# saegsali/visual-odometry-project

Measured on AMD Instinct MI355X. Metric: VO frames/sec at 1376x1241, 2k keypoints; pose err vs reference, higher is better.
Workload: dtype f64

## Files before the change

### visual-odometry-project_amd/csrc/pipeline.h

```cpp
#pragma once

#include <linux/futex.h>
#include <sys/prctl.h>
#include <sys/syscall.h>
#include <time.h>
#include <unistd.h>

#include <atomic>
#include <chrono>
#include <cmath>
#include <cstdlib>
#include <string>
#include <mutex>
#include <thread>
#include <vector>

#include "vo_state.h"
#include "state_device.h"

struct vo_pipeline_boot;

struct vo_pipeline {
  vo_ctx* ctx = nullptr;
  vo_ctx* det = nullptr;
// ... 27 lines not shown
  struct lens_t {
    bool on = false, have_raw = false;
    double dist[5] = {0, 0, 0, 0, 0}, K_raw[9] = {0, 0, 0, 0, 0, 0, 0, 0, 0};
  };
  std::vector<lens_t> lens;
  uint8_t* d_raw[2] = {nullptr, nullptr};
  uint8_t* h_bgr = nullptr;
  hipEvent_t evBgr = nullptr;
  int prepared_idx = -1, prepared_slot = -1;
  int slot = 0, det_flip = 0, prev_frame = -1;
  vo_feat F[2];
  void* feat_mem = nullptr;
  int cur = 0;
  vo_seq_ctl* d_ctl = nullptr;
  float *d_next = nullptr, *d_err = nullptr;
  uint8_t* d_status = nullptr;
  double *d_R = nullptr, *d_t = nullptr;
  uint8_t* d_valid = nullptr;
  int32_t *d_counts = nullptr, *d_samples = nullptr, *d_pend = nullptr;
  uint64_t *d_masks = nullptr, *d_best_mask = nullptr;
  double* d_table = nullptr;
  std::vector<double> table;
  int table_len = 0;
  uint32_t* d_raws = nullptr;
  uint32_t ring_len = 0;
  uint32_t* h_stage = nullptr;
  size_t stage_cap = 0;
  std::vector<uint64_t> gen_upto, pos_known, pos_dev;
  std::vector<vo_pcg64> raw_gen, rng;
  hipEvent_t evRaw = nullptr;
  bool raw_pending = false, seeded = false, have_state = false, primed = false;
  vo_step_result *h_res = nullptr, *m_res = nullptr;
  volatile unsigned* h_seq = nullptr;
  unsigned* m_seq = nullptr;
  unsigned seq = 0;
  struct flight_t { int prev_idx = 0, next_idx = 0, a = 0, b = 0, fcur = 0, rslot = 0; unsigned seq = 0; long k = 0; unsigned front_job = 0; };
  flight_t flight[2];
  int n_flight = 0;
  long steps_submitted = 0;
  std::vector<unsigned> slot_seq;
  std::vector<char> seq_state;
  int last_fbuf = 0;
  long last_k = 0;
  int ckpt_par = 0;
  hipEvent_t evA = nullptr, evB = nullptr;
  double* d_newkp = nullptr;
// ... 134 lines not shown
```

### visual-odometry-project_amd/csrc/pipeline.hip

```cpp
#include "pipeline.h"

#pragma clang fp contract(off)

namespace {

hipError_t mset(hipStream_t st, void* dst, int v, size_t bytes) {
  hipError_t e = hipMemsetAsync(dst, v, bytes, st);
  return e != hipSuccess ? e : hipStreamSynchronize(st);
}

uint32_t next_pow2(uint64_t v) {
  uint32_t r = 1;
  while (r < v) r <<= 1;
  return r;
}

vo_feat carve(char*& q, int cap, int S, bool ids) {
  vo_feat f;
  auto take = [&](size_t bytes) {
    void* r = q;
    q += (bytes * S + 255) & ~size_t(255);
    return r;
  };
  f.kp = (float*)take((size_t)cap * 8);
// ... 160 lines not shown
  VO_REQUIRE(ctx, cfg->track_ids == 0 || cfg->track_ids == 1, "pipeline: track_ids must be 0 (off) or 1 (on), got %d", cfg->track_ids);
  VO_REQUIRE(ctx, cfg->detector == 0 || cfg->tracker_mode == 0,
             "pipeline: the Shi-Tomasi detector (detector = 1) belongs to the KLT tracker mode (tracker_mode = 0)");
  if (cfg->detector == 1) {
    const int rc = vo_good_features_batch_check(ctx, cfg->sequences > 0 ? cfg->sequences : 1, cfg->H, cfg->W,
                                                cfg->st_quality == 0.0 ? 0.01 : cfg->st_quality,
                                                cfg->st_min_distance == 0.0 ? 8.0 : cfg->st_min_distance,
                                                cfg->st_block == 0 ? 7 : cfg->st_block);
    if (rc != VO_OK) return rc;
  }
  const int cap = cfg->feature_cap > 0 ? cfg->feature_cap : 2 * cfg->n_keypoints;
  VO_REQUIRE(ctx, cap >= cfg->n_keypoints && cap <= 32768, "pipeline: feature_cap must be in n_keypoints..32768");
  VO_HIP_TRY(ctx, hipSetDevice(ctx->device));
  vo_pipeline* p = new (std::nothrow) vo_pipeline();
  if (!p) return VO_ENOMEM;
  p->ctx = ctx;
  p->cfg = *cfg;
  p->cap = cap;
  p->words = vo_cdiv(cap, 64);
  p->S = cfg->sequences > 0 ? cfg->sequences : 1;
  p->cfg.sequences = p->S;
  const int S = p->S;
  if (p->cfg.bearing_threshold == 0.0) p->cfg.bearing_threshold = 0.0075;
  if (p->cfg.redetect_fraction == 0.0) p->cfg.redetect_fraction = 0.8;
  if (p->cfg.detect_margin == 0.0) p->cfg.detect_margin = 0.01;
  if (p->cfg.detect_losses <= 0.0) p->cfg.detect_losses = 2.5;
  if (p->cfg.st_block == 0) p->cfg.st_block = 7;
  if (p->cfg.st_quality == 0.0) p->cfg.st_quality = 0.01;
  if (p->cfg.st_min_distance == 0.0) p->cfg.st_min_distance = 8.0;
  p->detect_losses = p->cfg.detect_losses;
  p->detect_limit = p->cfg.detect_margin < 0.0 ? -1.0 : p->cfg.redetect_fraction + p->cfg.detect_margin;
  if (p->cfg.debug_never_detect) p->detect_limit = 0.0;
  {
    bool given = false;
    for (double v : cfg->Kinv) given |= v != 0.0;
    p->cams.assign((size_t)p->S, make_cam(cfg->K, given ? cfg->Kinv : nullptr));
  }
  p->idle.assign((size_t)p->S, 0);
  memset(&p->seed_rng, 0, sizeof(p->seed_rng));
  int rc = VO_OK;
  void* side = getenv("VO_ONE_STREAM") ? (void*)ctx->stream : nullptr;
  {
    const char* sc = getenv("VO_SIDE_CUS");
    p->side_cfg = vo_stream_cfg_parse(sc, getenv("VO_STREAM_PRIORITY"));
    if (!sc && p->S <= 2 && p->detect_limit >= 0.0 && !side && cfg->tracker_mode == 0) {
      hipDeviceProp_t prop;
// ... 366 lines not shown
```

### visual-odometry-project_amd/csrc/pipeline_state.hip

```cpp
#include <algorithm>

#include "pipeline.h"

#pragma clang fp contract(off)

namespace {

struct pose17 {
  double v[17];
};

__global__ __launch_bounds__(256) void export_state_kernel(pose17 head, const double* __restrict__ land, int n, int cap,
                                                           double* __restrict__ rec) {
  const int i = blockIdx.x * blockDim.x + threadIdx.x;
  if (i < 17) rec[i] = head.v[i];
  const int m = min(n, cap) * 3;
  if (i < m) rec[17 + i] = land[i];
}

__global__ __launch_bounds__(256) void export_tracks_kernel(vo_feat F, const vo_seq_ctl* __restrict__ ctl, int slot, int n,
                                                            int cap, int seq, unsigned long long* __restrict__ rec) {
  const int i = blockIdx.x * 256 + threadIdx.x;
  auto pack = [](int lo, int hi) { return (unsigned long long)(unsigned)lo | ((unsigned long long)(unsigned)hi << 32); };
  if (i == 0) {
// ... 452 lines not shown
    VO_HIP_TRY(ctx, hipMemcpyAsync(p->d_newkp, new_kp, (size_t)n2 * 16, hipMemcpyHostToDevice, st));
    VO_HIP_TRY(ctx, hipMemcpyAsync(p->d_pairs, pairs, (size_t)M * 8, hipMemcpyHostToDevice, st));
    vo_pairs_batch bt;
    bt.par = (int)(p->steps_submitted & 1);
    VO_TRY(vo_state_regroup_pairs(ctx, p->d_ctl, p->F[p->cur], p->F[1 - p->cur], p->d_pairs, M, p->d_newkp, n2, p->cap, nullptr,
                                  nullptr, nullptr, 1, &bt));
    VO_HIP_TRY(ctx, hipStreamSynchronize(st));
    p->cur = 1 - p->cur;
    vo_seq_ctl h;
    VO_HIP_TRY(ctx, mcpy(st, &h, p->d_ctl, sizeof(h), hipMemcpyDeviceToHost));
    memcpy(h.T_in_wc, T_wc, 96);
    memcpy(h.T_in_cw, T_cw, 96);
    h.n_cand = h.n_dropped = h.n_land = h.done = 0;
    h.next_id[bt.par] = h.next_id[bt.par ^ 1];
    h.id_step[bt.par] = h.id_step[bt.par ^ 1];
    VO_HIP_TRY(ctx, mcpy(st, p->d_ctl, &h, sizeof(h), hipMemcpyHostToDevice));
    std::vector<uint64_t> bits((size_t)p->words, ~0ull);
    if (p3p_inliers)
      for (int i = 0; i < h.n_tri; ++i)
        if (!p3p_inliers[i]) bits[i >> 6] &= ~(1ull << (i & 63));
    VO_HIP_TRY(ctx, mcpy(st, p->d_best_mask, bits.data(), bits.size() * 8, hipMemcpyHostToDevice));
  }
  if (phases & 1)
    VO_TRY(vo_state_candidates(ctx, p->d_ctl, p->F[p->cur], p->d_best_mask, p->d_cams, p->cfg.bearing_threshold, -1, p->cap));
  if (phases & 2)
    VO_TRY(vo_state_landmarks(ctx, p->d_ctl, p->F[p->cur], p->d_cams, -1, p->cap, nullptr, nullptr, 0u));
  VO_HIP_TRY(ctx, hipStreamSynchronize(st));
  return VO_OK;
}

int vo_pipeline_export_state_post_seq(vo_pipeline* p, int seq, const vo_step_result* r, int cap, double* d_record) {
  if (!p || !r || !d_record) return VO_EINVAL;
  vo_ctx* ctx = p->ctx;
  VO_REQUIRE(ctx, cap >= 0 && seq >= 0 && seq < p->S, "pipeline_export_state: bad capacity or sequence index");
  pose17 h;
  for (int row = 0; row < 3; ++row) {
    for (int c = 0; c < 3; ++c) h.v[4 * row + c] = r->R_refined[3 * row + c];
    h.v[4 * row + 3] = r->t_refined[row];
  }
  h.v[12] = h.v[13] = h.v[14] = 0.0;
  h.v[15] = 1.0;
  const int n = r->best_index >= 0 ? (r->n_triangulated < cap ? r->n_triangulated : cap) : 0;
  h.v[16] = (double)n;
  const int threads = n * 3 > 17 ? n * 3 : 17;
  {
    vo_prof_scope ps(ctx, VO_K_EXPORT);
    hipLaunchKernelGGL(export_state_kernel, dim3(vo_cdiv(threads, 256)), dim3(256), 0, ctx->stream, h,
// ... 129 lines not shown
```

### visual-odometry-project_amd/csrc/pipeline_step.hip

```cpp
#include "pipeline.h"

#pragma clang fp contract(off)

namespace {

__global__ __launch_bounds__(64) void detect_decide_kernel(const vo_seq_ctl* __restrict__ ctl, int S, double limit, int n_det,
                                                           int force, int* __restrict__ go, double losses) {
  const int q = blockIdx.x * 64 + threadIdx.x;
  if (q >= S) return;
  if (ctl[q].fault & VO_FAULT_IDLE) {
    go[q] = 0;
    return;
  }
  const int n2 = ctl[q].n2;
  const int lost = max(ctl[q].n_in - (ctl[q].redetected ? (n_det < 0 ? ctl[q].num_features : n_det) : 0) - n2, 0);
  go[q] = (force || limit < 0.0 || (limit > 0.0 && (double)n2 - losses * (double)lost < (double)ctl[q].num_features * limit)) ? 1 : 0;
}

__global__ void ctl_resume_kernel(vo_seq_ctl* __restrict__ ctl) {
  ctl->fault = 0;
  ctl->n_p3p = ctl->n_tri;
}

__global__ __launch_bounds__(256) void sift_kp_f64_kernel(const float* __restrict__ rows, const int* __restrict__ n, int cap,
// ... 152 lines not shown
  p->gen_upto[q] = target;
  return VO_OK;
}

static vo_pose_job make_pose_job(vo_pipeline* p, const vo_feat& B, int do_replay, int q0) {
  const vo_pipeline_config& c = p->cfg;
  const size_t q = (size_t)q0;
  vo_pose_job j;
  j.ctl = p->d_ctl + q;
  j.rp.valid = p->d_valid + q * c.hyp;
  j.rp.counts = p->d_counts + q * c.hyp;
  j.rp.R = p->d_R + q * c.hyp * 9;
  j.rp.t = p->d_t + q * c.hyp * 3;
  j.rp.masks = (const unsigned long long*)p->d_masks + q * c.hyp * p->words;
  j.rp.words = p->words;
  j.rp.hyp = c.hyp;
  j.rp.table = p->d_table;
  j.rp.table_len = p->table_len;
  j.rp.max_it = c.ransac_max_iterations;
  j.rp.best_mask = (unsigned long long*)p->d_best_mask + q * p->words;
  j.do_replay = do_replay;
  j.B = vo_feat_seq(B, q);
  j.cam = p->d_cams + q;
  j.bearing_thr = c.bearing_threshold;
  j.max_iter = c.refine_iters;
  j.tail = 0;
  j.res = nullptr;
  j.seq_word = nullptr;
  j.seq = 0u;
  static const int stamps = getenv("VO_POSE_STAMPS") ? 1 : 0;
  j.stamps = stamps;
  j.debug_fault_every = 0;
  return j;
}

static int enqueue_tracker(vo_pipeline* p, const vo_pipeline::flight_t& f, bool with_pyramid, int q0, int Sn) {
  vo_ctx* ctx = p->ctx;
  const vo_pipeline_config& c = p->cfg;
  const vo_feat A = vo_feat_seq(p->F[f.fcur], (size_t)q0);
  hipStream_t ts = p->trk->stream;
  if (with_pyramid) VO_TRY(enqueue_pyramid(p, f.next_idx, f.b));
  if (f.k > 0 && hipEventQuery(p->evRegroup[(f.k - 1) & 1]) != hipSuccess)
    VO_HIP_TRY(ctx, hipStreamWaitEvent(ts, p->evRegroup[(f.k - 1) & 1], 0));
  if (hipEventQuery(p->evDet[f.a]) != hipSuccess) VO_HIP_TRY(ctx, hipStreamWaitEvent(ts, p->evDet[f.a], 0));
  vo_seq_ctl* ctl = p->d_ctl + q0;
  vo_klt_source src;
  src.n = &ctl->n2;
// ... 64 lines not shown
  const size_t q = (size_t)q0;
  const vo_feat B = vo_feat_seq(p->F[1 - f.fcur], q);
  vo_seq_ctl* ctl = p->d_ctl + q0;
  vo_hyp_batch hb;
  hb.S = Sn;
  hb.X = (size_t)p->cap * 3;
  hb.x = (size_t)p->cap * 2;
  hb.raws = p->ring_len;
  hb.ctl = sizeof(vo_seq_ctl);
  hb.cam = reinterpret_cast<const double*>(p->d_cams + q);
  hb.cam_stride = sizeof(vo_cam) / sizeof(double);
  VO_TRY(vo_p3p_hypotheses_ring_dev(ctx, B.land, B.kp64, &ctl->n_p3p, p->cap, c.K, p->d_raws + q * p->ring_len, &ctl->raw_pos,
                                    p->ring_len - 1, c.hyp, c.p3p_thr_sq, p->d_R + q * c.hyp * 9, p->d_t + q * c.hyp * 3,
                                    p->d_valid + q * c.hyp, p->d_counts + q * c.hyp, p->d_masks + q * c.hyp * p->words,
                                    (uint32_t*)&ctl->solve_flag, (uint64_t*)&ctl->ts[2], &hb));
  vo_pose_job job = make_pose_job(p, p->F[1 - f.fcur], 1, q0);
  job.walk = 0;
  job.res = p->m_res + (size_t)f.rslot * p->S + q;
  job.seq_word = p->m_seq + (size_t)f.rslot * p->S + q;
  job.seq = seq;
  job.debug_fault_every = debug_pose_fault;
  VO_TRY(vo_frame_pose(ctx, job, Sn));
  const uint64_t* bm = p->d_best_mask + (size_t)q0 * p->words;
  return vo_state_walk_landmarks(ctx, ctl, B, bm, p->words, p->d_cams + q0, c.bearing_threshold, c.refine_iters > 0 ? 1 : 0,
                                 p->cap, p->d_pend + q * p->cap, job.res, job.seq_word, seq, Sn);
}

extern "C" int vo_sift_dev(vo_ctx* ctx, const uint8_t* d_img, int H, int W, int cap, float* d_kp, float* d_desc,
                           uint8_t* d_desc_u8, int32_t* d_n);

static int enqueue_sift(vo_pipeline* p, const vo_pipeline::flight_t& f, char* err_buf = nullptr) {
  vo_ctx* sc = (f.k & 1) ? p->det : p->trk;
  const vo_pipeline_config& c = p->cfg;
  int rc = VO_OK;
  if (sc != p->trk && hipStreamWaitEvent(sc->stream, p->evImg[f.next_idx], 0) != hipSuccess) rc = VO_EHIP;
  if (rc == VO_OK && p->n_pinned[f.next_idx] > 0 && hipStreamWaitEvent(sc->stream, p->evUp[f.next_idx], 0) != hipSuccess) rc = VO_EHIP;
  if (rc == VO_OK && p->sift_all)
    rc = vo_sift_all_found_dev(sc, p->img(0, f.next_idx), p->img_stride(), 1, c.H, c.W, p->frame_rows,
                               p->d_skp + (size_t)f.b * p->frame_rows * 6, (size_t)p->frame_rows, nullptr, p->frame_desc(f.b, 0),
                               (size_t)p->frame_rows, p->frame_n(f.b, 0), p->d_sover + 2 * f.b, p->d_sover + 2 * f.b + 1);
  else if (rc == VO_OK)
    rc = vo_sift_dev(sc, p->img(0, f.next_idx), c.H, c.W, p->frame_rows, p->d_skp + (size_t)f.b * p->frame_rows * 6, nullptr,
                     p->frame_desc(f.b, 0), p->frame_n(f.b, 0));
  if (rc == VO_OK && hipEventRecord(p->evPyr[f.b], sc->stream) != hipSuccess) rc = VO_EHIP;
  return rc != VO_OK ? launch_error(p, err_buf, rc, "sift", vo_last_error(sc)) : VO_OK;
}

// ... 556 lines not shown
```

### visual-odometry-project_amd/csrc/refine.hip

```cpp
#include <type_traits>
#include "state_device.h"
#include "dlt_device.h"

#pragma clang fp contract(off)

namespace {

constexpr int RF_T = 512;
constexpr int RF_S = 28;
constexpr int RF_W = 29;
constexpr int RF_PT = 4;

struct rf_point {
  double X, Y, Z, u, v;
  bool on;
};

__device__ __forceinline__ rf_point load_point(const double* __restrict__ X, const double* __restrict__ x, int N,
                                               const uint8_t* __restrict__ mask8,
                                               const unsigned long long* __restrict__ mask_bits, int i) {
  rf_point p;
  const bool in = i < N;
  const int j = in ? i : 0;
  p.X = X[3 * j];
// ... 408 lines not shown
    if (tid == 0) {
      ctl->n_cand = 0;
      ctl->n_pend = 0;
    }
    return;
  }
  double Tcw[12], Twc[12];
#pragma unroll
  for (int r = 0; r < 3; ++r) {
    Tcw[4 * r] = s_pose[3 * r];
    Tcw[4 * r + 1] = s_pose[3 * r + 1];
    Tcw[4 * r + 2] = s_pose[3 * r + 2];
    Tcw[4 * r + 3] = s_pose[9 + r];
  }
  rigid_inverse_3x4(Tcw, Twc);
  const int n2 = ctl->n2, n_tri = ctl->n_tri;
  if (tid == 0) {
    s_nc = 0;
    s_tail[0] = s_tail[1] = 0;
  }
  __syncthreads();
  int count = 0;
  for (int i = tid; i < n2; i += RF_T) {
    const int c = candidate_feature(job.B, i, n_tri, mask_bits, *job.cam, Twc, job.bearing_thr);
    count += c;
    if (c && job.tail) {
      const int slot = atomicAdd(&s_nc, 1);
      if (slot < TAIL_LIST) s_list[slot] = i;
    }
  }
  count = wave_sum_i32(count);
  if (lane == 0) s_cand[wv] = count;
  __syncthreads();
  int n_cand = 0;
  for (int w = 0; w < RF_T / 64; ++w) n_cand += s_cand[w];
  if (tid == 0) {
    ctl->n_cand = n_cand;
    ctl->n = n2;
  }
  if (tid < 12) {
    double ncw = 0.0, nwc = 0.0;
#pragma unroll
    for (int k = 0; k < 12; ++k) {
      ncw = tid == k ? Tcw[k] : ncw;
      nwc = tid == k ? Twc[k] : nwc;
    }
    commit_pose(ctl, tid, ncw, nwc);
// ... 164 lines not shown
```

### visual-odometry-project_amd/csrc/state.hip

```cpp
#include <cmath>

#include "dlt_device.h"
#include "state_device.h"

#pragma clang fp contract(off)

namespace {

constexpr int RG_T = 1024;


using namespace vo_state_dev;

__device__ __forceinline__ unsigned long long block_scan_excl(unsigned long long v, unsigned long long* s_wave,
                                                              unsigned long long* total) {
  const int lane = threadIdx.x & 63, wv = threadIdx.x >> 6, nw = blockDim.x >> 6;
  unsigned long long inc = v;
#pragma unroll
  for (int off = 1; off < 64; off <<= 1) {
    const unsigned long long o = __shfl_up(inc, off);
    if (lane >= off) inc += o;
  }
  if (lane == 63) s_wave[wv] = inc;
  __syncthreads();
// ... 376 lines not shown
    ctl->det_ran = ap.det_go ? ap.det_go[blockIdx.y] : 1;
    if (ap.n_det_dev) {
      const int nf_next = redetect ? n_det : nf;
      ctl->nf[ap.nf_par ^ 1] = nf_next;
      ctl->num_features = nf_next;
    }
    if (IDS) {
      ctl->next_id[ap.nf_par ^ 1] = nid + (n_in - n);
      ctl->id_step[ap.nf_par ^ 1] = step_k + 1;
    }
    ctl->n2 = T0 + T1 + T2;
    ctl->n_tri = T0;
    ctl->n_mat = T1;
    ctl->n_new = T2;
    const int few = T0 < 8 ? VO_FAULT_FEW_LANDMARKS : 0;
    ctl->n_p3p = few ? 0 : T0;
    ctl->few = few;
  }
}


__global__ __launch_bounds__(256) void state_candidates_kernel(vo_seq_ctl* __restrict__ ctl, vo_feat B,
                                                               const unsigned long long* __restrict__ best_mask,
                                                               const vo_cam* __restrict__ cams, double bearing_thr, int use_refined,
                                                               int words) {
  if (blockIdx.y != 0) {
    const size_t q = blockIdx.y;
    ctl += q;
    B = vo_feat_seq(B, q);
    best_mask += q * (size_t)words;
  }
  const vo_cam& cam = cams[blockIdx.y];
  if (ctl->fault) return;
  const int tid = threadIdx.x;
  const int n2 = ctl->n2, n_tri = ctl->n_tri;
  double Tcw[12], Twc[12];
  if (use_refined < 0) {
#pragma unroll
    for (int k = 0; k < 12; ++k) Tcw[k] = ctl->T_in_cw[k];
#pragma unroll
    for (int k = 0; k < 12; ++k) Twc[k] = ctl->T_in_wc[k];
  } else {
    const double* src = use_refined ? ctl->refined : ctl->best_pose;
#pragma unroll
    for (int r = 0; r < 3; ++r) {
      Tcw[4 * r] = src[3 * r];
      Tcw[4 * r + 1] = src[3 * r + 1];
      Tcw[4 * r + 2] = src[3 * r + 2];
      Tcw[4 * r + 3] = src[9 + r];
    }
    rigid_inverse_3x4(Tcw, Twc);
  }
  const int i = blockIdx.x * 256 + tid;
  const int cand = i < n2 ? candidate_feature(B, i, n_tri, best_mask, cam, Twc, bearing_thr) : 0;
  const unsigned long long cm = __ballot(cand != 0);
  if ((tid & 63) == 0 && cm) atomicAdd(&ctl->n_cand, __popcll(cm));
  if (blockIdx.x == 0) {
    if (tid < 12) {
      double ncw = 0.0, nwc = 0.0;
#pragma unroll
      for (int k = 0; k < 12; ++k) {
        ncw = tid == k ? Tcw[k] : ncw;
        nwc = tid == k ? Twc[k] : nwc;
      }
      commit_pose(ctl, tid, ncw, nwc);
    }
    if (tid == 0) ctl->n = n2;
  }
}

__global__ __launch_bounds__(256) void state_landmarks_kernel(vo_seq_ctl* __restrict__ ctl, vo_feat B, const vo_cam* __restrict__ cams,
                                                              int use_refined, vo_step_result* __restrict__ res,
                                                              unsigned* __restrict__ seq_word, unsigned seq) {
  __shared__ int s_cnt[2];
  __shared__ int s_last;
  const int tid = threadIdx.x;
  if (blockIdx.y != 0) {
// ... 63 lines not shown
    if ((tid & 63) == 0) {
      if (d) atomicAdd(&s_cnt[0], d);
      if (l) atomicAdd(&s_cnt[1], l);
    }
  }
  __syncthreads();
  if (tid == 0) {
    if (s_cnt[0]) atomicAdd(&ctl->n_dropped, s_cnt[0]);
    if (s_cnt[1]) atomicAdd(&ctl->n_land, s_cnt[1]);
    __threadfence();
    s_last = atomicAdd(&ctl->done, 1) == (int)gridDim.x - 1 ? 1 : 0;
  }
  __syncthreads();
  if (!s_last) return;
  const int n_dropped = atomicAdd(&ctl->n_dropped, 0), n_land = atomicAdd(&ctl->n_land, 0);
  if (tid == 0) ctl->step += 1;
  if (!res) return;
  write_step_record(ctl, tid, use_refined, n2, n_cand, n_dropped, n_land, atomicAdd(&ctl->ts[4], 0ull), res, seq_word, seq);
}


__global__ __launch_bounds__(256) void state_walk_landmarks_kernel(vo_seq_ctl* __restrict__ ctl, vo_feat B,
                                                                   const unsigned long long* __restrict__ best_mask, int words,
                                                                   const vo_cam* __restrict__ cams, double bearing_thr, int use_refined,
                                                                   int* __restrict__ pend, vo_step_result* __restrict__ res,
                                                                   unsigned* __restrict__ seq_word, unsigned seq) {
  __shared__ int s_cnt[3];
  __shared__ int s_last;
  const int tid = threadIdx.x;
  if (blockIdx.y != 0) {
    const size_t q = blockIdx.y;
    ctl += q;
    pend += q * (size_t)B.pitch;
    B = vo_feat_seq(B, q);
    best_mask += q * (size_t)words;
    if (res) {
      res += q;
      seq_word += q;
    }
  }
  if (blockIdx.x == 0 && tid == 0) ctl->ts[4] = wall_clock64();
  const vo_cam& cam = cams[blockIdx.y];
  const int fault = ctl->fault;
  if (fault) {
    if (res && blockIdx.x == 0 && tid == 0) write_fault_record(ctl, fault, res, seq_word, seq);
    return;
  }
  const int n2 = ctl->n2, n_tri = ctl->n_tri;
  if (tid < 3) s_cnt[tid] = 0;
  double Tcw[12], Twc[12], Tp[12];
#pragma unroll
  for (int r = 0; r < 3; ++r) {
    Tcw[4 * r] = ctl->refined[3 * r];
    Tcw[4 * r + 1] = ctl->refined[3 * r + 1];
    Tcw[4 * r + 2] = ctl->refined[3 * r + 2];
    Tcw[4 * r + 3] = ctl->refined[9 + r];
  }
  rigid_inverse_3x4(Tcw, Twc);
#pragma unroll
  for (int k = 0; k < 12; ++k) Tp[k] = ctl->T_cw[k];
  __syncthreads();
  const int i = blockIdx.x * 256 + tid;
  int cand = 0, st = 0;
  double X[3] = {0.0, 0.0, 0.0};
// ... 15 lines not shown
      reset = true;
    }
    if (reset) {
      if (st0 != 0) {
        B.track[2 * i] = u;
        B.track[2 * i + 1] = v;
        B.state[i] = 0;
      }
#pragma unroll
      for (int k = 0; k < 12; ++k) B.pose[(size_t)k * B.pitch + i] = Twc[k];
      st = 0;
    } else if (st == 1) {
      const double* Ki = cam.Kinv;
      const double n1x = Ki[0] * ta + Ki[1] * tb + Ki[2], n1y = Ki[3] * ta + Ki[4] * tb + Ki[5],
                   n1z = Ki[6] * ta + Ki[7] * tb + Ki[8];
      const double n2x = Ki[0] * u + Ki[1] * v + Ki[2], n2y = Ki[3] * u + Ki[4] * v + Ki[5],
                   n2z = Ki[6] * u + Ki[7] * v + Ki[8];
      const double r1x = Ts[0] * n1x + Ts[1] * n1y + Ts[2] * n1z, r1y = Ts[4] * n1x + Ts[5] * n1y + Ts[6] * n1z,
                   r1z = Ts[8] * n1x + Ts[9] * n1y + Ts[10] * n1z;
      const double r2x = Twc[0] * n2x + Twc[1] * n2y + Twc[2] * n2z, r2y = Twc[4] * n2x + Twc[5] * n2y + Twc[6] * n2z,
                   r2z = Twc[8] * n2x + Twc[9] * n2y + Twc[10] * n2z;
      const double dot = r1x * r2x + r1y * r2y + r1z * r2z;
      const double l1 = sqrt(r1x * r1x + r1y * r1y + r1z * r1z), l2 = sqrt(r2x * r2x + r2y * r2y + r2z * r2z);
      const double ang = acos(dot / (l1 * l2));
      cand = ang >= bearing_thr ? 1 : 0;
    }
    B.cand[i] = (uint8_t)cand;
    if (cand) {
      double Ti[12], C1[12], C2[12];
      rigid_inverse_3x4(Ts, Ti);
      k_times(cam.K, Ti, C1);
      k_times(cam.K, Tcw, C2);
      vo_dlt::triangulate_point(C1, ta, tb, C2, u, v, X);
      B.land[3 * i] = X[0];
      B.land[3 * i + 1] = X[1];
      B.land[3 * i + 2] = X[2];
      st = 2;
      B.state[i] = 2;
    }
  }
  {
    const unsigned long long cm = __ballot(cand != 0);
    if ((tid & 63) == 0 && cm) atomicAdd(&s_cnt[2], __popcll(cm));
  }
  __syncthreads();
  const int local_cand = s_cnt[2];
  auto drop = [&](int f) {
    const double nan = dnan();
    B.land[3 * f] = B.land[3 * f + 1] = B.land[3 * f + 2] = nan;
    B.state[f] = 0;
    B.track[2 * f] = B.kp64[2 * f];
    B.track[2 * f + 1] = B.kp64[2 * f + 1];
#pragma unroll
    for (int k = 0; k < 12; ++k) B.pose[(size_t)k * B.pitch + f] = Twc[k];
  };
  int dropped = 0;
  if (i < n2) {
    const double zc = Tcw[8] * X[0] + Tcw[9] * X[1] + Tcw[10] * X[2] + Tcw[11];
    const double zp = Tp[8] * X[0] + Tp[9] * X[1] + Tp[10] * X[2] + Tp[11];
    if (zc < 0.0 || zp < 0.0) {
      if (local_cand > 0) {
        drop(i);
        st = 0;
        dropped = 1;
      } else {
        pend[atomicAdd(&ctl->n_pend, 1)] = i;
      }
    }
  }
  {
    const int d = __popcll(__ballot(dropped != 0)), l = __popcll(__ballot(i < n2 && st == 2));
    if ((tid & 63) == 0) {
      if (d) atomicAdd(&s_cnt[0], d);
      if (l) atomicAdd(&s_cnt[1], l);
    }
  }
  __syncthreads();
  if (tid == 0) {
    if (s_cnt[0]) atomicAdd(&ctl->n_dropped, s_cnt[0]);
    if (s_cnt[1]) atomicAdd(&ctl->n_land, s_cnt[1]);
    if (local_cand) atomicAdd(&ctl->n_cand, local_cand);
    __threadfence();
    s_last = atomicAdd(&ctl->done, 1) == (int)gridDim.x - 1 ? 1 : 0;
  }
  __syncthreads();
  if (!s_last) return;
  __threadfence();
  const int n_cand = atomicAdd(&ctl->n_cand, 0), n_pend = atomicAdd(&ctl->n_pend, 0);
  int n_dropped = atomicAdd(&ctl->n_dropped, 0), n_land = atomicAdd(&ctl->n_land, 0);
  if (n_cand > 0 && n_pend > 0) {
    if (tid < 2) s_cnt[tid] = 0;
    __syncthreads();
    for (int k = tid; k < n_pend; k += 256) {
      const int f = pend[k];
      if (B.state[f] == 2) atomicAdd(&s_cnt[1], 1);
      drop(f);
      atomicAdd(&s_cnt[0], 1);
    }
    __syncthreads();
    n_dropped += s_cnt[0];
    n_land -= s_cnt[1];
  }
  if (tid < 12) {
    double ncw = 0.0, nwc = 0.0;
#pragma unroll
    for (int k = 0; k < 12; ++k) {
      ncw = tid == k ? Tcw[k] : ncw;
      nwc = tid == k ? Twc[k] : nwc;
    }
    commit_pose(ctl, tid, ncw, nwc);
  }
  if (tid == 0) {
    ctl->n = n2;
    ctl->step += 1;
  }
  if (!res) return;
  __syncthreads();
  write_step_record(ctl, tid, use_refined, n2, n_cand, n_dropped, n_land, atomicAdd(&ctl->ts[4], 0ull), res, seq_word, seq,
                    false);
}

}

int vo_state_regroup_klt(vo_ctx* ctx, vo_seq_ctl* ctl, vo_feat A, vo_feat B, const float* d_next_xy,
                         const uint8_t* d_status, const float* d_err, float err_thr, vo_append ap, int cap, int S) {
  {
    vo_prof_scope ps(ctx, VO_K_STATE_REGROUP);
    if (A.ids)
      vo_launch_stop(ctx, state_regroup_klt_kernel<true>, dim3(vo_cdiv(cap, 256), S), dim3(256), 0, ctx->stream, ctl, A, B,
                     d_next_xy, d_status, d_err, err_thr, ap, cap);
    else
      vo_launch_stop(ctx, state_regroup_klt_kernel<false>, dim3(vo_cdiv(cap, 256), S), dim3(256), 0, ctx->stream, ctl, A, B,
                     d_next_xy, d_status, d_err, err_thr, ap, cap);
  }
  return vo_check_launch(ctx, "state_regroup_klt_kernel");
}

int vo_state_regroup_pairs(vo_ctx* ctx, vo_seq_ctl* ctl, vo_feat A, vo_feat B, const int32_t* d_pairs, int M,
                           const double* d_new_kp, int n2_in, int cap, const int32_t* d_M, const int32_t* d_n2,
                           int32_t* d_src_row, int S, const vo_pairs_batch* batch) {
  VO_REQUIRE(ctx, cap <= RG_T * RG_MAX_PER && n2_in <= cap && M <= cap, "state_regroup: capacity exceeded");
  VO_REQUIRE(ctx, S >= 1 && (S == 1 || batch), "state_regroup: several sequences need their strides");
  const vo_pairs_batch bt = batch ? *batch : vo_pairs_batch{};
  {
    vo_prof_scope ps(ctx, VO_K_STATE_REGROUP);
    auto kernel = A.ids ? state_regroup_kernel<true, true> : state_regroup_kernel<true, false>;
    hipLaunchKernelGGL(kernel, dim3(S), dim3(RG_T), 0, ctx->stream, ctl, A, B, (const float*)nullptr,
                       (const uint8_t*)nullptr, (const float*)nullptr, 0.f, d_pairs, M, d_new_kp, n2_in, cap,
                       (const int*)d_M, (const int*)d_n2, (int*)d_src_row, bt);
  }
  return vo_check_launch(ctx, "state_regroup_kernel");
}

int vo_state_candidates(vo_ctx* ctx, vo_seq_ctl* ctl, vo_feat B, const uint64_t* d_best_mask, const vo_cam* d_cams,
                        double bearing_thr, int use_refined, int cap, int S, int words) {
  {
    vo_prof_scope ps(ctx, VO_K_STATE_CANDIDATES);
    hipLaunchKernelGGL(state_candidates_kernel, dim3(vo_cdiv(cap, 256), S), dim3(256), 0, ctx->stream, ctl, B,
                       (const unsigned long long*)d_best_mask, d_cams, bearing_thr, use_refined, words);
  }
  return vo_check_launch(ctx, "state_candidates_kernel");
}

int vo_state_walk_landmarks(vo_ctx* ctx, vo_seq_ctl* ctl, vo_feat B, const uint64_t* d_best_mask, int words, const vo_cam* d_cams,
                            double bearing_thr, int use_refined, int cap, int32_t* d_pend, vo_step_result* m_result,
                            unsigned* m_seq, unsigned seq, int S) {
  VO_REQUIRE(ctx, d_pend != nullptr && cap <= B.pitch, "state_walk_landmarks: bad arguments");
  {
    vo_prof_scope ps(ctx, VO_K_STATE_LANDMARKS);
    hipLaunchKernelGGL(state_walk_landmarks_kernel, dim3(vo_cdiv(cap, 256), S), dim3(256), 0, ctx->stream, ctl, B,
                       (const unsigned long long*)d_best_mask, words, d_cams, bearing_thr, use_refined, (int*)d_pend, m_result,
                       m_seq, seq);
  }
  return vo_check_launch(ctx, "state_walk_landmarks_kernel");
}

int vo_state_landmarks(vo_ctx* ctx, vo_seq_ctl* ctl, vo_feat B, const vo_cam* d_cams, int use_refined, int cap,
                       vo_step_result* m_result, unsigned* m_seq, unsigned seq, int S) {
  {
    vo_prof_scope ps(ctx, VO_K_STATE_LANDMARKS);
    hipLaunchKernelGGL(state_landmarks_kernel, dim3(vo_cdiv(cap, 256), S), dim3(256), 0, ctx->stream, ctl, B, d_cams,
                       use_refined, m_result, m_seq, seq);
  }
  return vo_check_launch(ctx, "state_landmarks_kernel");
}

int64_t vo_ransac_table_lookup(const double* table, int table_len, int64_t max_iterations, double outlier_ratio) {
  return (int64_t)vo_state_dev::table_lookup(table, table_len, (long long)max_iterations, outlier_ratio);
}

void vo_ransac_build_table(double confidence, int s, int table_len, double* table) {
  auto f = [&](double o) { return (double)vo_ransac_num_iterations(confidence, o, s); };
  const double kmin = f(0.01);
  table[0] = kmin;
  const double fmax_ = f(0.99);
  double lo_start = 0.01;
  for (int j = 0; j < table_len; ++j) {
    const double target = kmin + j + 1;
    if (fmax_ < target) {
      table[1 + j] = INFINITY;
      continue;
    }
    uint64_t lo, hi;
    double a = lo_start, b = 0.99;
    memcpy(&lo, &a, 8);
    memcpy(&hi, &b, 8);
    if (f(a) >= target) {
// ... 17 lines not shown
```

### visual-odometry-project_amd/csrc/state_device.h

```cpp
#pragma once
#include <cstddef>
#include "vo_state.h"

#pragma clang fp contract(off)

namespace vo_state_dev {

__device__ __forceinline__ double dnan() { return __longlong_as_double(0x7ff8000000000000ll); }

__device__ __forceinline__ void rigid_inverse_3x4(const double* T, double* Ti) {
#pragma unroll
  for (int r = 0; r < 3; ++r) {
#pragma unroll
    for (int c = 0; c < 3; ++c) Ti[4 * r + c] = T[4 * c + r];
    Ti[4 * r + 3] = -(T[r] * T[3] + T[4 + r] * T[7] + T[8 + r] * T[11]);
  }
}

__device__ __forceinline__ void k_times(const double* K, const double* T, double* C) {
#pragma unroll
  for (int r = 0; r < 3; ++r)
#pragma unroll
    for (int c = 0; c < 4; ++c) C[4 * r + c] = K[3 * r] * T[c] + K[3 * r + 1] * T[4 + c] + K[3 * r + 2] * T[8 + c];
}
// ... 162 lines not shown
      if (lds_mask) s_mask[w] = m;
    }
  } else if (!more) {
    if (s_best && lane < 12) s_best[lane] = ctl->best_pose[lane];
    if (lds_mask)
      for (int w = lane; w < wn; w += 64) s_mask[w] = a.best_mask[w];
  }
  if (s_mask_ok && lane == 0) *s_mask_ok = lds_mask ? 1 : 0;
  if (lane == 0) {
    if (more) consumed = hyp;
    ctl->n_iterations = n_it;
    ctl->outlier_ratio = orat;
    ctl->raw_pos += 7ull * (unsigned long long)consumed;
    ctl->best_idx = best_idx >= 0 ? cont * hyp + best_idx : best_idx_before;
    ctl->best_count = best;
    ctl->consumed = consumed_before + consumed;
    ctl->hyp_valid = hyp_valid;
    ctl->n_done = n;
    ctl->cont = more ? cont + 1 : 0;
    if (more) ctl->fault = VO_FAULT_CONTINUE;
  }
}

__device__ __forceinline__ int candidate_feature(const vo_feat& B, int i, int n_tri,
                                                 const unsigned long long* __restrict__ best_mask, const vo_cam& cam,
                                                 const double* Twc, double bearing_thr, int* st_out = nullptr) {
  int st = B.state[i];
  const int st0 = st;
  const double u = B.kp64[2 * i], v = B.kp64[2 * i + 1];
  bool reset = st == 0;
  if (i < n_tri && !((best_mask[i >> 6] >> (i & 63)) & 1ull)) {
    st = 0;
    reset = true;
  }
  int cand = 0;
  if (reset) {
    if (st0 != 0) {
      B.track[2 * i] = u;
      B.track[2 * i + 1] = v;
      B.state[i] = 0;
    }
#pragma unroll
    for (int k = 0; k < 12; ++k) B.pose[(size_t)k * B.pitch + i] = Twc[k];
  } else if (st == 1) {
    double P[11];
#pragma unroll
    for (int k = 0; k < 11; ++k) P[k] = B.pose[(size_t)k * B.pitch + i];
    const double a = B.track[2 * i], b = B.track[2 * i + 1];
    const double* Ki = cam.Kinv;
    const double n1x = Ki[0] * a + Ki[1] * b + Ki[2], n1y = Ki[3] * a + Ki[4] * b + Ki[5],
                 n1z = Ki[6] * a + Ki[7] * b + Ki[8];
    const double n2x = Ki[0] * u + Ki[1] * v + Ki[2], n2y = Ki[3] * u + Ki[4] * v + Ki[5],
                 n2z = Ki[6] * u + Ki[7] * v + Ki[8];
    const double r1x = P[0] * n1x + P[1] * n1y + P[2] * n1z, r1y = P[4] * n1x + P[5] * n1y + P[6] * n1z,
                 r1z = P[8] * n1x + P[9] * n1y + P[10] * n1z;
    const double r2x = Twc[0] * n2x + Twc[1] * n2y + Twc[2] * n2z, r2y = Twc[4] * n2x + Twc[5] * n2y + Twc[6] * n2z,
                 r2z = Twc[8] * n2x + Twc[9] * n2y + Twc[10] * n2z;
    const double dot = r1x * r2x + r1y * r2y + r1z * r2z;
    const double l1 = sqrt(r1x * r1x + r1y * r1y + r1z * r1z), l2 = sqrt(r2x * r2x + r2y * r2y + r2z * r2z);
    const double ang = acos(dot / (l1 * l2));
    cand = ang >= bearing_thr ? 1 : 0;
  }
  B.cand[i] = (uint8_t)cand;
  if (st_out) *st_out = reset ? 0 : st;
  return cand;
}

__device__ __forceinline__ void commit_pose(vo_seq_ctl* __restrict__ ctl, int tid, double ncw, double nwc) {
  const double ocw = ctl->T_cw[tid], owc = ctl->T_wc[tid];
  ctl->T_cw_prev[tid] = ocw;
  ctl->T_wc_prev[tid] = owc;
  ctl->T_cw[tid] = ncw;
  ctl->T_wc[tid] = nwc;
}

constexpr int REC_DW = (int)(sizeof(vo_step_result) / 4);
static_assert(sizeof(vo_step_result) % 4 == 0 && REC_DW <= 128 + 2, "record: two dwords per lane of one wave");
static_assert(offsetof(vo_step_result, seq_head) == sizeof(vo_step_result) - 8 &&
              offsetof(vo_step_result, seq_tail) == sizeof(vo_step_result) - 4, "record: the closing words come last");

__host__ __device__ inline unsigned record_mix(unsigned v, int k) {
  return (v + 0x9e3779b9u * (unsigned)(k + 1)) * (unsigned)(2 * k + 1);
}

// ... 92 lines not shown
```

### visual-odometry-project_amd/csrc/vo_state.h

```cpp
#pragma once
#include "vo_internal.h"

struct vo_feat {
  float* kp;
  double* kp64;
  uint8_t* state;
  uint8_t* cand;
  double* land;
  double* track;
  double* pose;
  int pitch;
  int2* ids = nullptr;
};

__host__ __device__ inline vo_feat vo_feat_seq(vo_feat F, size_t q) {
  const size_t n = q * (size_t)F.pitch;
  F.kp += 2 * n;
  F.kp64 += 2 * n;
  F.state += n;
  F.cand += n;
  F.land += 3 * n;
  F.track += 2 * n;
  F.pose += 12 * n;
  if (F.ids) F.ids += n;
// ... 56 lines not shown
  const int* det_go;
  const int32_t* n_det_dev = nullptr;
  int nf_par = 0;
};

struct vo_replay_args {
  const uint8_t* valid;
  const int32_t* counts;
  const double *R, *t;
  const unsigned long long* masks;
  int words, hyp;
  const double* table;
  int table_len;
  long long max_it;
  unsigned long long* best_mask;
};

struct vo_pose_job {
  vo_seq_ctl* ctl;
  vo_replay_args rp;
  int do_replay;
  vo_feat B;
  const vo_cam* cam;
  double bearing_thr;
  int max_iter;
  int tail;
  vo_step_result* res;
  unsigned* seq_word;
  unsigned seq;
  int stamps;
  int walk = 1;
  int debug_fault_every;
};
int vo_frame_pose(vo_ctx* ctx, const vo_pose_job& job, int S = 1);

int vo_state_regroup_klt(vo_ctx* ctx, vo_seq_ctl* ctl, vo_feat A, vo_feat B, const float* d_next_xy,
                         const uint8_t* d_status, const float* d_err, float err_thr, vo_append ap, int cap, int S = 1);
struct vo_pairs_batch {
  size_t pairs = 0;
  size_t new_kp = 0;
  size_t src_row = 0;
  int M = 0, n2 = 0;
  int debug_fault_every = 0;
  int par = 0;
};
int vo_state_regroup_pairs(vo_ctx* ctx, vo_seq_ctl* ctl, vo_feat A, vo_feat B, const int32_t* d_pairs, int M,
                           const double* d_new_kp, int n2_in, int cap, const int32_t* d_M = nullptr,
                           const int32_t* d_n2 = nullptr, int32_t* d_src_row = nullptr, int S = 1,
                           const vo_pairs_batch* batch = nullptr);
int vo_state_candidates(vo_ctx* ctx, vo_seq_ctl* ctl, vo_feat B, const uint64_t* d_best_mask, const vo_cam* d_cams,
                        double bearing_thr, int use_refined, int cap, int S = 1, int words = 0);
int vo_state_walk_landmarks(vo_ctx* ctx, vo_seq_ctl* ctl, vo_feat B, const uint64_t* d_best_mask, int words, const vo_cam* d_cams,
                            double bearing_thr, int use_refined, int cap, int32_t* d_pend, vo_step_result* m_result,
                            unsigned* m_seq, unsigned seq, int S);
int vo_state_landmarks(vo_ctx* ctx, vo_seq_ctl* ctl, vo_feat B, const vo_cam* d_cams, int use_refined, int cap,
                       vo_step_result* m_result, unsigned* m_seq, unsigned seq, int S = 1);
int64_t vo_ransac_table_lookup(const double* table, int table_len, int64_t max_iterations, double outlier_ratio);
void vo_ransac_build_table(double confidence, int s, int table_len, double* table);
```

Baseline: 10910.

## Replace per-feature acos bearing test with precomputed cosine limit; relax landmark-walk fences

Precomputes on the host, by bisection over double bit patterns, the largest cosine value whose acos still meets the bearing threshold. Device candidate tests then compare the normalized dot product against that limit instead of calling acos per feature. Separately, the walk-landmarks kernel swaps __threadfence and atomicAdd-of-zero reads for relaxed agent-scope atomics and explicit vmcnt waits. It also packs the landmark-state bit into the pending index so the last block no longer rereads B.state. This removes transcendental work and heavier fences, at the risk of subtle memory-ordering or boundary-equivalence issues.

New measurement: 10990, median of 3. About the same (+0.8%).

```diff
diff --git a/visual-odometry-project_amd/csrc/pipeline.h b/visual-odometry-project_amd/csrc/pipeline.h
--- a/visual-odometry-project_amd/csrc/pipeline.h
+++ b/visual-odometry-project_amd/csrc/pipeline.h
@@ -73,6 +73,7 @@
   double* d_table = nullptr;
   std::vector<double> table;
   int table_len = 0;
+  double bearing_x_lim = 1.0;
   uint32_t* d_raws = nullptr;
   uint32_t ring_len = 0;
   uint32_t* h_stage = nullptr;
diff --git a/visual-odometry-project_amd/csrc/pipeline.hip b/visual-odometry-project_amd/csrc/pipeline.hip
--- a/visual-odometry-project_amd/csrc/pipeline.hip
+++ b/visual-odometry-project_amd/csrc/pipeline.hip
@@ -206,6 +206,7 @@
   p->cfg.sequences = p->S;
   const int S = p->S;
   if (p->cfg.bearing_threshold == 0.0) p->cfg.bearing_threshold = 0.0075;
+  p->bearing_x_lim = vo_bearing_x_limit(p->cfg.bearing_threshold);
   if (p->cfg.redetect_fraction == 0.0) p->cfg.redetect_fraction = 0.8;
   if (p->cfg.detect_margin == 0.0) p->cfg.detect_margin = 0.01;
   if (p->cfg.detect_losses <= 0.0) p->cfg.detect_losses = 2.5;
diff --git a/visual-odometry-project_amd/csrc/pipeline_state.hip b/visual-odometry-project_amd/csrc/pipeline_state.hip
--- a/visual-odometry-project_amd/csrc/pipeline_state.hip
+++ b/visual-odometry-project_amd/csrc/pipeline_state.hip
@@ -498,7 +498,7 @@
     VO_HIP_TRY(ctx, mcpy(st, p->d_best_mask, bits.data(), bits.size() * 8, hipMemcpyHostToDevice));
   }
   if (phases & 1)
-    VO_TRY(vo_state_candidates(ctx, p->d_ctl, p->F[p->cur], p->d_best_mask, p->d_cams, p->cfg.bearing_threshold, -1, p->cap));
+    VO_TRY(vo_state_candidates(ctx, p->d_ctl, p->F[p->cur], p->d_best_mask, p->d_cams, p->bearing_x_lim, -1, p->cap));
   if (phases & 2)
     VO_TRY(vo_state_landmarks(ctx, p->d_ctl, p->F[p->cur], p->d_cams, -1, p->cap, nullptr, nullptr, 0u));
   VO_HIP_TRY(ctx, hipStreamSynchronize(st));
diff --git a/visual-odometry-project_amd/csrc/pipeline_step.hip b/visual-odometry-project_amd/csrc/pipeline_step.hip
--- a/visual-odometry-project_amd/csrc/pipeline_step.hip
+++ b/visual-odometry-project_amd/csrc/pipeline_step.hip
@@ -198,7 +198,7 @@
   j.do_replay = do_replay;
   j.B = vo_feat_seq(B, q);
   j.cam = p->d_cams + q;
-  j.bearing_thr = c.bearing_threshold;
+  j.bearing_x_lim = p->bearing_x_lim;
   j.max_iter = c.refine_iters;
   j.tail = 0;
   j.res = nullptr;
@@ -309,7 +309,7 @@
   job.debug_fault_every = debug_pose_fault;
   VO_TRY(vo_frame_pose(ctx, job, Sn));
   const uint64_t* bm = p->d_best_mask + (size_t)q0 * p->words;
-  return vo_state_walk_landmarks(ctx, ctl, B, bm, p->words, p->d_cams + q0, c.bearing_threshold, c.refine_iters > 0 ? 1 : 0,
+  return vo_state_walk_landmarks(ctx, ctl, B, bm, p->words, p->d_cams + q0, p->bearing_x_lim, c.refine_iters > 0 ? 1 : 0,
                                  p->cap, p->d_pend + q * p->cap, job.res, job.seq_word, seq, Sn);
 }
 
diff --git a/visual-odometry-project_amd/csrc/refine.hip b/visual-odometry-project_amd/csrc/refine.hip
--- a/visual-odometry-project_amd/csrc/refine.hip
+++ b/visual-odometry-project_amd/csrc/refine.hip
@@ -454,7 +454,7 @@
   __syncthreads();
   int count = 0;
   for (int i = tid; i < n2; i += RF_T) {
-    const int c = candidate_feature(job.B, i, n_tri, mask_bits, *job.cam, Twc, job.bearing_thr);
+    const int c = candidate_feature(job.B, i, n_tri, mask_bits, *job.cam, Twc, job.bearing_x_lim);
     count += c;
     if (c && job.tail) {
       const int slot = atomicAdd(&s_nc, 1);
diff --git a/visual-odometry-project_amd/csrc/state.hip b/visual-odometry-project_amd/csrc/state.hip
--- a/visual-odometry-project_amd/csrc/state.hip
+++ b/visual-odometry-project_amd/csrc/state.hip
@@ -422,7 +422,7 @@
 
 __global__ __launch_bounds__(256) void state_candidates_kernel(vo_seq_ctl* __restrict__ ctl, vo_feat B,
                                                                const unsigned long long* __restrict__ best_mask,
-                                                               const vo_cam* __restrict__ cams, double bearing_thr, int use_refined,
+                                                               const vo_cam* __restrict__ cams, double x_lim, int use_refined,
                                                                int words) {
   if (blockIdx.y != 0) {
     const size_t q = blockIdx.y;
@@ -452,7 +452,7 @@
     rigid_inverse_3x4(Tcw, Twc);
   }
   const int i = blockIdx.x * 256 + tid;
-  const int cand = i < n2 ? candidate_feature(B, i, n_tri, best_mask, cam, Twc, bearing_thr) : 0;
+  const int cand = i < n2 ? candidate_feature(B, i, n_tri, best_mask, cam, Twc, x_lim) : 0;
   const unsigned long long cm = __ballot(cand != 0);
   if ((tid & 63) == 0 && cm) atomicAdd(&ctl->n_cand, __popcll(cm));
   if (blockIdx.x == 0) {
@@ -562,7 +562,7 @@
 
 __global__ __launch_bounds__(256) void state_walk_landmarks_kernel(vo_seq_ctl* __restrict__ ctl, vo_feat B,
                                                                    const unsigned long long* __restrict__ best_mask, int words,
-                                                                   const vo_cam* __restrict__ cams, double bearing_thr, int use_refined,
+                                                                   const vo_cam* __restrict__ cams, double x_lim, int use_refined,
                                                                    int* __restrict__ pend, vo_step_result* __restrict__ res,
                                                                    unsigned* __restrict__ seq_word, unsigned seq) {
   __shared__ int s_cnt[3];
@@ -579,7 +579,8 @@
       seq_word += q;
     }
   }
-  if (blockIdx.x == 0 && tid == 0) ctl->ts[4] = wall_clock64();
+  if (blockIdx.x == 0 && tid == 0)
+    __hip_atomic_store(&ctl->ts[4], (unsigned long long)wall_clock64(), __ATOMIC_RELAXED, __HIP_MEMORY_SCOPE_AGENT);
   const vo_cam& cam = cams[blockIdx.y];
   const int fault = ctl->fault;
   if (fault) {
@@ -641,8 +642,7 @@
                    r2z = Twc[8] * n2x + Twc[9] * n2y + Twc[10] * n2z;
       const double dot = r1x * r2x + r1y * r2y + r1z * r2z;
       const double l1 = sqrt(r1x * r1x + r1y * r1y + r1z * r1z), l2 = sqrt(r2x * r2x + r2y * r2y + r2z * r2z);
-      const double ang = acos(dot / (l1 * l2));
-      cand = ang >= bearing_thr ? 1 : 0;
+      cand = bearing_candidate(dot / (l1 * l2), x_lim);
     }
     B.cand[i] = (uint8_t)cand;
     if (cand) {
@@ -674,6 +674,7 @@
     for (int k = 0; k < 12; ++k) B.pose[(size_t)k * B.pitch + f] = Twc[k];
   };
   int dropped = 0;
+  bool pending = false;
   if (i < n2) {
     const double zc = Tcw[8] * X[0] + Tcw[9] * X[1] + Tcw[10] * X[2] + Tcw[11];
     const double zp = Tp[8] * X[0] + Tp[9] * X[1] + Tp[10] * X[2] + Tp[11];
@@ -683,10 +684,13 @@
         st = 0;
         dropped = 1;
       } else {
-        pend[atomicAdd(&ctl->n_pend, 1)] = i;
+        pending = true;
+        __hip_atomic_store(&pend[atomicAdd(&ctl->n_pend, 1)], 2 * i + (st == 2 ? 1 : 0), __ATOMIC_RELAXED,
+                           __HIP_MEMORY_SCOPE_AGENT);
       }
     }
   }
+  if (__ballot(pending) != 0ull) asm volatile("s_waitcnt vmcnt(0)" ::: "memory");
   {
     const int d = __popcll(__ballot(dropped != 0)), l = __popcll(__ballot(i < n2 && st == 2));
     if ((tid & 63) == 0) {
@@ -699,20 +703,23 @@
     if (s_cnt[0]) atomicAdd(&ctl->n_dropped, s_cnt[0]);
     if (s_cnt[1]) atomicAdd(&ctl->n_land, s_cnt[1]);
     if (local_cand) atomicAdd(&ctl->n_cand, local_cand);
-    __threadfence();
+    asm volatile("s_waitcnt vmcnt(0)" ::: "memory");
     s_last = atomicAdd(&ctl->done, 1) == (int)gridDim.x - 1 ? 1 : 0;
   }
   __syncthreads();
   if (!s_last) return;
-  __threadfence();
-  const int n_cand = atomicAdd(&ctl->n_cand, 0), n_pend = atomicAdd(&ctl->n_pend, 0);
-  int n_dropped = atomicAdd(&ctl->n_dropped, 0), n_land = atomicAdd(&ctl->n_land, 0);
+  const int n_cand = __hip_atomic_load(&ctl->n_cand, __ATOMIC_RELAXED, __HIP_MEMORY_SCOPE_AGENT),
+            n_pend = __hip_atomic_load(&ctl->n_pend, __ATOMIC_RELAXED, __HIP_MEMORY_SCOPE_AGENT);
+  int n_dropped = __hip_atomic_load(&ctl->n_dropped, __ATOMIC_RELAXED, __HIP_MEMORY_SCOPE_AGENT),
+      n_land = __hip_atomic_load(&ctl->n_land, __ATOMIC_RELAXED, __HIP_MEMORY_SCOPE_AGENT);
+  const unsigned long long ts4 = __hip_atomic_load(&ctl->ts[4], __ATOMIC_RELAXED, __HIP_MEMORY_SCOPE_AGENT);
   if (n_cand > 0 && n_pend > 0) {
     if (tid < 2) s_cnt[tid] = 0;
     __syncthreads();
     for (int k = tid; k < n_pend; k += 256) {
-      const int f = pend[k];
-      if (B.state[f] == 2) atomicAdd(&s_cnt[1], 1);
+      const int w = __hip_atomic_load(&pend[k], __ATOMIC_RELAXED, __HIP_MEMORY_SCOPE_AGENT);
+      const int f = w >> 1;
+      if (w & 1) atomicAdd(&s_cnt[1], 1);
       drop(f);
       atomicAdd(&s_cnt[0], 1);
     }
@@ -735,7 +742,7 @@
   }
   if (!res) return;
   __syncthreads();
-  write_step_record(ctl, tid, use_refined, n2, n_cand, n_dropped, n_land, atomicAdd(&ctl->ts[4], 0ull), res, seq_word, seq,
+  write_step_record(ctl, tid, use_refined, n2, n_cand, n_dropped, n_land, ts4, res, seq_word, seq,
                     false);
 }
 
@@ -772,23 +779,23 @@
 }
 
 int vo_state_candidates(vo_ctx* ctx, vo_seq_ctl* ctl, vo_feat B, const uint64_t* d_best_mask, const vo_cam* d_cams,
-                        double bearing_thr, int use_refined, int cap, int S, int words) {
+                        double bearing_x_lim, int use_refined, int cap, int S, int words) {
   {
     vo_prof_scope ps(ctx, VO_K_STATE_CANDIDATES);
     hipLaunchKernelGGL(state_candidates_kernel, dim3(vo_cdiv(cap, 256), S), dim3(256), 0, ctx->stream, ctl, B,
-                       (const unsigned long long*)d_best_mask, d_cams, bearing_thr, use_refined, words);
+                       (const unsigned long long*)d_best_mask, d_cams, bearing_x_lim, use_refined, words);
   }
   return vo_check_launch(ctx, "state_candidates_kernel");
 }
 
 int vo_state_walk_landmarks(vo_ctx* ctx, vo_seq_ctl* ctl, vo_feat B, const uint64_t* d_best_mask, int words, const vo_cam* d_cams,
-                            double bearing_thr, int use_refined, int cap, int32_t* d_pend, vo_step_result* m_result,
+                            double bearing_x_lim, int use_refined, int cap, int32_t* d_pend, vo_step_result* m_result,
                             unsigned* m_seq, unsigned seq, int S) {
   VO_REQUIRE(ctx, d_pend != nullptr && cap <= B.pitch, "state_walk_landmarks: bad arguments");
   {
     vo_prof_scope ps(ctx, VO_K_STATE_LANDMARKS);
     hipLaunchKernelGGL(state_walk_landmarks_kernel, dim3(vo_cdiv(cap, 256), S), dim3(256), 0, ctx->stream, ctl, B,
-                       (const unsigned long long*)d_best_mask, words, d_cams, bearing_thr, use_refined, (int*)d_pend, m_result,
+                       (const unsigned long long*)d_best_mask, words, d_cams, bearing_x_lim, use_refined, (int*)d_pend, m_result,
                        m_seq, seq);
   }
   return vo_check_launch(ctx, "state_walk_landmarks_kernel");
@@ -802,6 +809,28 @@
                        use_refined, m_result, m_seq, seq);
   }
   return vo_check_launch(ctx, "state_landmarks_kernel");
+}
+
+double vo_bearing_x_limit(double thr) {
+  auto ok = [thr](double x) {
+    volatile double a = std::acos(x);
+    return a >= thr;
+  };
+  if (ok(1.0)) return 1.0;
+  if (!ok(-1.0)) return -2.0;
+  const bool neg = !ok(0.0);
+  auto at = [neg](uint64_t bits) {
+    double x;
+    memcpy(&x, &bits, 8);
+    return neg ? -x : x;
+  };
+  uint64_t good = neg ? 0x3ff0000000000000ull : 0ull, bad = neg ? 0ull : 0x3ff0000000000000ull;
+  while ((good > bad ? good - bad : bad - good) > 1ull) {
+    const uint64_t mid = good / 2 + bad / 2 + (good & bad & 1ull);
+    if (ok(at(mid))) good = mid;
+    else bad = mid;
+  }
+  return at(good);
 }
 
 int64_t vo_ransac_table_lookup(const double* table, int table_len, int64_t max_iterations, double outlier_ratio) {
diff --git a/visual-odometry-project_amd/csrc/state_device.h b/visual-odometry-project_amd/csrc/state_device.h
--- a/visual-odometry-project_amd/csrc/state_device.h
+++ b/visual-odometry-project_amd/csrc/state_device.h
@@ -208,9 +208,11 @@
   }
 }
 
+__device__ __forceinline__ int bearing_candidate(double x, double x_lim) { return (x >= -1.0 && x <= x_lim) ? 1 : 0; }
+
 __device__ __forceinline__ int candidate_feature(const vo_feat& B, int i, int n_tri,
                                                  const unsigned long long* __restrict__ best_mask, const vo_cam& cam,
-                                                 const double* Twc, double bearing_thr, int* st_out = nullptr) {
+                                                 const double* Twc, double x_lim, int* st_out = nullptr) {
   int st = B.state[i];
   const int st0 = st;
   const double u = B.kp64[2 * i], v = B.kp64[2 * i + 1];
@@ -244,8 +246,7 @@
                  r2z = Twc[8] * n2x + Twc[9] * n2y + Twc[10] * n2z;
     const double dot = r1x * r2x + r1y * r2y + r1z * r2z;
     const double l1 = sqrt(r1x * r1x + r1y * r1y + r1z * r1z), l2 = sqrt(r2x * r2x + r2y * r2y + r2z * r2z);
-    const double ang = acos(dot / (l1 * l2));
-    cand = ang >= bearing_thr ? 1 : 0;
+    cand = bearing_candidate(dot / (l1 * l2), x_lim);
   }
   B.cand[i] = (uint8_t)cand;
   if (st_out) *st_out = reset ? 0 : st;
diff --git a/visual-odometry-project_amd/csrc/vo_state.h b/visual-odometry-project_amd/csrc/vo_state.h
--- a/visual-odometry-project_amd/csrc/vo_state.h
+++ b/visual-odometry-project_amd/csrc/vo_state.h
@@ -102,7 +102,7 @@
   int do_replay;
   vo_feat B;
   const vo_cam* cam;
-  double bearing_thr;
+  double bearing_x_lim;
   int max_iter;
   int tail;
   vo_step_result* res;
@@ -128,10 +128,11 @@
                            const double* d_new_kp, int n2_in, int cap, const int32_t* d_M = nullptr,
                            const int32_t* d_n2 = nullptr, int32_t* d_src_row = nullptr, int S = 1,
                            const vo_pairs_batch* batch = nullptr);
+double vo_bearing_x_limit(double bearing_thr);
 int vo_state_candidates(vo_ctx* ctx, vo_seq_ctl* ctl, vo_feat B, const uint64_t* d_best_mask, const vo_cam* d_cams,
-                        double bearing_thr, int use_refined, int cap, int S = 1, int words = 0);
+                        double bearing_x_lim, int use_refined, int cap, int S = 1, int words = 0);
 int vo_state_walk_landmarks(vo_ctx* ctx, vo_seq_ctl* ctl, vo_feat B, const uint64_t* d_best_mask, int words, const vo_cam* d_cams,
-                            double bearing_thr, int use_refined, int cap, int32_t* d_pend, vo_step_result* m_result,
+                            double bearing_x_lim, int use_refined, int cap, int32_t* d_pend, vo_step_result* m_result,
                             unsigned* m_seq, unsigned seq, int S);
 int vo_state_landmarks(vo_ctx* ctx, vo_seq_ctl* ctl, vo_feat B, const vo_cam* d_cams, int use_refined, int cap,
                        vo_step_result* m_result, unsigned* m_seq, unsigned seq, int S = 1);
```
